# sczhou/CodeFormer

Measured on AMD Instinct MI355X. Metric: aligned 512x512 faces/sec (whole node) at w=0.5, higher is better.
Workload: dtype f32; 1 GPU; BASELINE config 2 (IEEE fp32 arithmetic): 16 faces/GPU, w=0.5, adain, seed-0 random-init weights; global_batch=16, parallelism=single GPU, precision=fp32

## Files before the change

### codeformer_amd/archs/codeformer_arch.py

```python
import gc
import os
import threading

import math
import numbers

import numpy as np
import torch
import torch.nn.functional as F
from torch import nn

from .. import ops
from ..ops import EPI_GELU, EPI_RESIDUAL, EPI_SFT, PRO_LEAKY
from ..utils.diagnostics import top2_gap
from ..utils.registry import ARCH_REGISTRY
from .hip_module import PACK_EPOCH, HipModule
from .vqgan_arch import ResBlock, VQAutoEncoder


_GRAPH_LOCK = threading.RLock()
_CAPTURE_STREAMS = {}


def _min_nan(a, b):
# ... 96 lines not shown
    normalized = (content_feat - content_mean.expand(size)) / content_std.expand(size)
    return normalized * style_std.expand(size) + style_mean.expand(size)


class TransformerSALayer(HipModule):

    def __init__(self, embed_dim, nhead=8, dim_mlp=2048, dropout=0.0, activation='gelu'):
        super().__init__()
        if activation != 'gelu':
            raise RuntimeError(f'activation should be gelu for the MI355X path, not {activation}.')
        self.self_attn = nn.MultiheadAttention(embed_dim, nhead, dropout=dropout)
        self.linear1 = nn.Linear(embed_dim, dim_mlp)
        self.dropout = nn.Dropout(dropout)
        self.linear2 = nn.Linear(dim_mlp, embed_dim)
        self.norm1 = nn.LayerNorm(embed_dim)
        self.norm2 = nn.LayerNorm(embed_dim)
        self.dropout1 = nn.Dropout(dropout)
        self.dropout2 = nn.Dropout(dropout)
        self.embed_dim, self.nhead = embed_dim, nhead

    def with_pos_embed(self, tensor, pos):
        return tensor if pos is None else tensor + pos

    def forward_tokens(self, X, pos, batch, code=0, code_ln=None):
        E, H = self.embed_dim, self.nhead
        sa = self.self_attn
        w, b = sa.in_proj_weight, sa.in_proj_bias
        code_ln = code if code_ln is None else code_ln
        c1 = ln_code(self, self.norm1, code_ln, pos)
        c2 = ln_code(self, self.norm2, code_ln)
        c_o = code or bounded_code(self, 'o', code_ln, self.norm1, w[2 * E:], b[2 * E:])
        c_d = code or bounded_code(self, 'd', code_ln, self.norm2, self.linear1.weight, self.linear1.bias)
        pw_o = self._pw_conv(sa.out_proj, bf16=c_o)
        if pos is not None:
            t2, t2p = ops.layernorm(X, self.norm1.weight, self.norm1.bias, self.norm1.eps, pos=pos)
        else:
            t2 = t2p = ops.layernorm(X, self.norm1.weight, self.norm1.bias, self.norm1.eps)
        if c1 == ops.GSPLIT and (2 * E) % 128 == 0:
            pw_qkv = self._packed(('qkv', c1), lambda: ops.pack_weight(w, b, bf16=c1), w, b)
            qkv = ops.linear(t2p, pw_qkv, x_alt=t2, alt_from=2 * E)
            q, k, v = qkv[:, :E], qkv[:, E:2 * E], qkv[:, 2 * E:]
        else:
            pw_qk = self._packed(('qk', c1), lambda: ops.pack_weight(w[:2 * E], b[:2 * E], bf16=c1), w, b)
            pw_v = self._packed(('v', c1), lambda: ops.pack_weight(w[2 * E:], b[2 * E:], bf16=c1), w, b)
            qk = ops.linear(t2p, pw_qk)
            v = ops.linear(t2, pw_v)
            q, k = qk[:, :E], qk[:, E:]
        hd = E // H
        a = ops.attention(q, k, v, batch, H, hd, float(hd) ** -0.5)
        X = ops.linear(a, pw_o, epilogue=EPI_RESIDUAL, res=X)
        t2 = ops.layernorm(X, self.norm2.weight, self.norm2.bias, self.norm2.eps)
        h = ops.linear(t2, self._pw_conv('linear1', bf16=c2), epilogue=EPI_GELU)
        return ops.linear(h, self._pw_conv('linear2', bf16=c_d), epilogue=EPI_RESIDUAL, res=X)

    def forward(self, tgt, tgt_mask=None, tgt_key_padding_mask=None, query_pos=None):
        if tgt.is_cuda:
            if tgt_mask is not None or tgt_key_padding_mask is not None:
                raise NotImplementedError('attention masks are not part of the CodeFormer inference path')
            with torch.no_grad():
                T, B, E = tgt.shape
                X = tgt.float().transpose(0, 1).contiguous().view(B * T, E)
# ... 82 lines not shown
@ARCH_REGISTRY.register()
class CodeFormer(VQAutoEncoder):

    def __init__(self, dim_embd=512, n_head=8, n_layers=9, codebook_size=1024, latent_size=256,
                 connect_list=['32', '64', '128', '256'], fix_modules=['quantize', 'generator'], vqgan_path=None):
        super().__init__(512, 64, [1, 2, 2, 4, 4, 8], 'nearest', 2, [16], codebook_size)
        if vqgan_path is not None:
            self.load_state_dict(torch.load(vqgan_path, map_location='cpu')['params_ema'])
        if fix_modules is not None:
            for name in fix_modules:
                for p in getattr(self, name).parameters():
                    p.requires_grad = False

        self.precision = os.environ.get('CODEFORMER_HIP_PRECISION', 'f16x2')
        self.bf16_storage = os.environ.get('CODEFORMER_HIP_BF16_STORAGE', '1') != '0'
        self.winograd_f43_encoder = os.environ.get('CODEFORMER_HIP_F43_ENCODER', '1') == '1'
        self.logit_guard = os.environ.get('CODEFORMER_HIP_LOGIT_GUARD', 'off')
        self.logit_guard_gap = float(os.environ.get('CODEFORMER_HIP_LOGIT_GUARD_GAP', '1.1e-4'))
        self.reset_guard_stats()
        self.encoder_precision = os.environ.get('CODEFORMER_HIP_ENCODER_PRECISION', 'auto')
        self.gemm_precision = os.environ.get('CODEFORMER_HIP_GEMM_PRECISION', 'auto')
        self.use_hip_graphs = {'0': False, '1': True}.get(os.environ.get('CODEFORMER_HIP_GRAPHS', 'auto'), 'auto')
        self.graph_max_batch = 4
        self._graphs = {}
        self.graph_captures = 0
        self.connect_list = connect_list
        self.n_layers = n_layers
        self.n_head = n_head
        self.dim_embd = dim_embd
        self.dim_mlp = dim_embd * 2
        self.latent_size = latent_size

        self.position_emb = nn.Parameter(torch.zeros(latent_size, self.dim_embd))
        self.feat_emb = nn.Linear(256, self.dim_embd)
        self.ft_layers = nn.Sequential(*[
            TransformerSALayer(embed_dim=dim_embd, nhead=n_head, dim_mlp=self.dim_mlp, dropout=0.0)
            for _ in range(self.n_layers)])
        self.idx_pred_layer = nn.Sequential(nn.LayerNorm(dim_embd), nn.Linear(dim_embd, codebook_size, bias=False))

        self.channels = {'16': 512, '32': 256, '64': 256, '128': 128, '256': 128, '512': 64}
        self.fuse_encoder_block = {'512': 2, '256': 5, '128': 8, '64': 11, '32': 14, '16': 18}
        self.fuse_generator_block = {'16': 6, '32': 9, '64': 12, '128': 15, '256': 18, '512': 21}
        self.fuse_convs_dict = nn.ModuleDict()
        for f_size in self.connect_list:
            ch = self.channels[f_size]
            self.fuse_convs_dict[f_size] = Fuse_sft_block(ch, ch)
# ... 4 lines not shown
        else:
            B, _, Himg, Wimg = x.shape
            if (Himg, Wimg) != (512, 512):
                raise ValueError(f'CodeFormer expects aligned 512x512 faces, got {Himg}x{Wimg}')
            x = x.float().contiguous()
        enc_feat = {}
        enc_taps = {self.fuse_encoder_block[f]: (lambda t: enc_feat.__setitem__(str(t.shape[2]), t))
                    for f in self.connect_list}
        if self.encoder_precision not in ('auto', 'fp32', 'f16x2'):
            raise ValueError(f"encoder_precision must be 'auto', 'fp32' or 'f16x2', got {self.encoder_precision!r}")
        enc_code = ops.SPLIT if self.encoder_precision == 'f16x2' or (self.encoder_precision == 'auto' and self.precision != 'fp32') else ops.WINOGRAD
        if self.winograd_f43_encoder if f43_encoder is None else f43_encoder:
            enc_code = {ops.SPLIT: ops.SPLIT_F43, ops.WINOGRAD: ops.WINOGRAD_F43K}[enc_code]
        lq = self.encoder.forward_nhwc(x, enc_taps, bf16=enc_code, img_u8=u8)
        T = lq.shape[1] * lq.shape[2]
        tokens = lq.view(B * T, lq.shape[3])

        if self.gemm_precision not in ('auto', 'fp32', 'f16x2'):
            raise ValueError(f"gemm_precision must be 'auto', 'fp32' or 'f16x2', got {self.gemm_precision!r}")
        gcode = ops.GSPLIT if self.gemm_precision == 'f16x2' else 0
        gcode_ln = ops.GSPLIT if (self.gemm_precision == 'f16x2' or (self.gemm_precision == 'auto' and self.precision != 'fp32' and self.encoder_precision != 'fp32')) else 0
        X = ops.linear(tokens, self._pw_conv('feat_emb', bf16=gcode))
        for layer in self.ft_layers:
            X = layer.forward_tokens(X, self.position_emb, B, code=gcode, code_ln=gcode_ln)
        ln, head = self.idx_pred_layer[0], self.idx_pred_layer[1]
        logits2d = ops.linear(ops.layernorm(X, ln.weight, ln.bias, ln.eps), self._pw_conv(head, bf16=ln_code(self, ln, gcode_ln)))
        res = {'logits': logits2d.view(B, T, -1), 'lq_feat': ops.to_nchw(lq), 'idx': None, 'quant': None, 'enc_feat': enc_feat}
        if guard:
            idx, _, self.last_min_gap = ops.argmax_rows_gap(logits2d, T)
            res['idx'] = idx.view(B, T)
        if code_only:
            return res

        if not guard:
            idx = ops.argmax_rows(logits2d)
            res['idx'] = idx.view(B, T)
        quant = ops.codebook_gather(idx, self.quantize.embedding.weight, B, T,
                                    lq=tokens.view(B, T, -1) if adain else None)
        res['quant'] = quant.view(B, lq.shape[1], lq.shape[2], -1)
        if self.precision not in ('fp32', 'f16x2', 'bf16', 'fp16'):
            raise ValueError(f"precision must be 'fp32', 'f16x2', 'bf16' or 'fp16', got {self.precision!r}")
        return res

    def _generate_hip(self, quant, enc_feat, w, u8=False, out_u8=None):
        B = quant.shape[0]
        bf16 = {'fp32': ops.WINOGRAD_F43K,'f16x2': ops.SPLIT_F43, 'bf16': 1, 'fp16': 2}[self.precision]
        gen_taps = None
# ... 76 lines not shown
            return self._generate_host(quant, enc_feat, w)
        if w.none_fused:
            return self._generate_host(quant, enc_feat, 0.0)
        wt = torch.tensor(w.host, dtype=torch.float32)
        if w.all_fused:
            return self._generate_host(quant, enc_feat, wt)
        rf, ru = w.rows_fused, w.rows_unfused
        of = self._generate_host(quant[rf], {f: t[rf] for f, t in enc_feat.items()}, wt[rf])
        ou = self._generate_host(quant[ru], None, 0.0)
        out = of.new_empty((quant.shape[0],) + tuple(of.shape[1:]))
        out[rf] = of
        out[ru] = ou
        return out

    def _forward_host(self, x, w, detach_16, code_only, adain):
        logits, lq_feat, quant, enc_feat = self._encode_host(x, detach_16, code_only, adain)
        if code_only:
            return logits, lq_feat
        return self._generate_rows_host(quant, enc_feat, w), logits, lq_feat

    def _forward_graphed(self, x, w, code_only, adain, guard=False, u8=False, out_u8=None):
        with _GRAPH_LOCK:
            per_face = isinstance(w, FaceWeights)
            key = (tuple(x.shape), ('per-face', w.fused) if per_face else float(w), bool(code_only), bool(adain), self.precision, bool(self.bf16_storage), self.encoder_precision, self.gemm_precision, bool(self.winograd_f43_encoder), str(x.device), ops.switches(), bool(guard), bool(u8))
            ent = self._graphs.get(key)
            sig = self._param_signature()
            if ent is None or ent['epoch'] != PACK_EPOCH[0] or ent['sig'] != sig:
                static_x = x.clone() if u8 else x.float().contiguous().clone()
                for _ in range(2):
                    self._forward_hip(static_x, w, code_only, adain, guard=guard, u8=u8)
                torch.cuda.synchronize(x.device)
                graph = torch.cuda.CUDAGraph()
                cap = _CAPTURE_STREAMS.get(str(x.device))
                if cap is None:
                    cap = _CAPTURE_STREAMS[str(x.device)] = torch.cuda.Stream(device=x.device)
                with torch.cuda.stream(cap):
                    ops._act_cells(x.device, 4 * max(int(x.shape[0]), 1))
                    ops._counters(x.device, 4096)
                    if self.precision == 'fp32':
                        ops._kpart_ws(x.device, max(int(x.shape[0]), 1) << 20)
                cap.synchronize()
                gc_on = gc.isenabled()
                gc.disable()
                try:
                    with torch.cuda.graph(graph, stream=cap):
                        outs = self._forward_hip(static_x, w, code_only, adain, guard=guard, u8=u8)
                finally:
# ... 240 lines not shown
```

### codeformer_amd/csrc/cf_conv_parts.h

```cpp
#pragma once
#include <type_traits>

#include "cf_common.h"

int cf_winograd_launch(const cf_conv_desc* d, hipStream_t stream, int* parts_query, const float* sft_w_img = nullptr);
bool cf_wsplit_covers(const cf_conv_desc* d);
int cf_wsplit_launch(const cf_conv_desc* d, hipStream_t stream, int* parts_query, const float* sft_w_img = nullptr);
int cf_wf43_launch(const cf_conv_desc* d, hipStream_t stream, int* parts_query, const float* sft_w_img = nullptr);
int cf_ksum_launch(const cf_conv_desc* d, hipStream_t stream, const float* sft_w_img);
bool cf_wf43_k32(int cout, int cin);
int cf_split_launch(const cf_conv_desc* d, hipStream_t stream, int* parts_query, const float* sft_w_img = nullptr);
int cf_gemm_split_launch(const cf_conv_desc* d, hipStream_t stream, int* parts_query);
int cf_gemm_f32_tile_try(const cf_conv_desc* d, hipStream_t stream);
int cf_gemm_split_geometry(const cf_conv_desc* d, int* tiles, long* bytes_per_part);
int cf_winograd_splitk_geometry(const cf_conv_desc* d, int* tiles, long* bytes_per_part);
int cf_split_splitk_geometry(const cf_conv_desc* d, int* tiles, long* bytes_per_part);

template <class A>
inline void cf_fill_conv_args(A& a, const cf_conv_desc* d, const float* sft_w_img = nullptr) {
  a.in0 = d->in0;
  a.in1 = d->in1;
  a.c0 = d->c0;
  a.c1 = d->c1;
  a.cin = d->c0 + d->c1;
  a.batch = d->batch;
  a.cout = d->cout;
  a.prologue = d->prologue;
  a.epilogue = d->epilogue;
  a.pro_scale = d->pro_scale;
  a.pro_shift = d->pro_shift;
  a.weight = d->weight;
  a.bias = d->bias;
  a.res = d->res;
  a.sft_scale = d->sft_scale;
  a.sft_w = d->sft_w;
  a.sft_w_img = sft_w_img;
// ... 156 lines not shown
```

### codeformer_amd/csrc/cf_gemm_split.hip

```cpp
#include <cstdlib>
#include <type_traits>

#include "cf_conv_parts.h"

namespace {

struct GsArgs {
  const float* a;
  const float* w;
  const float* bias;
  const float* res;
  float* out;
  int M, N, K;
  int epilogue;
  float acc_scale;
  float* ws;
  unsigned* counters;
  int nsplit;
  const float* a_alt;
  int n_alt;
};
__device__ __forceinline__ const float* gs_rows(const GsArgs& g, int n0) { return (g.a_alt && n0 >= g.n_alt) ? g.a_alt : g.a; }

__device__ __forceinline__ float gs_bias(const GsArgs& g, int n) { return g.bias ? g.bias[n] : 0.f; }
// ... 296 lines not shown
        for (int r = 0; r < 16; ++r) gs_part[(((c * MI + mi) * NI + ni) * 16 + r) * 64 + lane] = acc[mi][ni][r];
  }
  __syncthreads();
#pragma unroll
  for (int ni = 0; ni < NI; ++ni) {
    const int n = n0 + ni * 32 + l31;
    const float bias = gs_bias(g, n);
#pragma unroll
    for (int mi = 0; mi < MI; ++mi)
#pragma unroll
      for (int j = 0; j < 4; ++j) {
        const int r = wave + 4 * j;
        float tot = 0.f;
        for (int c = 0; c < V; ++c) tot += gs_part[(((c * MI + mi) * NI + ni) * 16 + r) * 64 + lane];
        const size_t o = (size_t)(m0 + mi * 32 + cf_acc_row(r, lane)) * g.N + n;
        float v = tot * g.acc_scale + bias;
        if (g.epilogue == CF_EPI_GELU) v = 0.5f * v * (1.0f + erff(v * 0.70710678118654752440f));
        if (g.epilogue == CF_EPI_RESIDUAL) v += g.res[o];
        g.out[o] = v;
      }
  }
}

__global__ __launch_bounds__(256) void gemm_f32_tile_kernel(const GsArgs g) {
  __shared__ __attribute__((aligned(16))) float As[2][2][128][16];
  const int tid = threadIdx.x, lane = tid & 63, wave = __builtin_amdgcn_readfirstlane(tid >> 6);
  const int wm = wave >> 1, wn = wave & 1;
  const int half = lane >> 5, l31 = lane & 31;
  const int ntn = g.N / 64;
  const int nt = blockIdx.x % ntn, mt = blockIdx.x / ntn;
  const int m0 = mt * 128, n0 = nt * 64 + wn * 32;
  const int nst = g.K >> 5;

  const float* const asrc = gs_rows(g, n0) + (size_t)(m0 + (tid >> 3)) * g.K + (tid & 7) * 4;
  f32x4 rg[4][4];
  auto load_stage = [&](int st, auto buf) __attribute__((always_inline)) {
    constexpr int BUF = decltype(buf)::value;
#pragma unroll
    for (int j = 0; j < 4; ++j) rg[BUF][j] = *reinterpret_cast<const f32x4*>(asrc + (size_t)(32 * j) * g.K + st * 32);
  };
  auto store_stage = [&](int lbuf, auto buf) __attribute__((always_inline)) {
    constexpr int BUF = decltype(buf)::value;
    const int q = tid & 7, ks = q >> 2, ch = q & 3;
#pragma unroll
    for (int j = 0; j < 4; ++j) {
      const int row = (tid >> 3) + 32 * j;
      *reinterpret_cast<f32x4*>(&As[lbuf][ks][row][(ch ^ ((row >> 2) & 3)) << 2]) = rg[BUF][j];
    }
  };
  const float* const wl = g.w + (size_t)(n0 + l31) * 16 + half * 4;
  const size_t kstride = (size_t)g.N * 16;
  f32x4 rb[4][2][2];
  auto load_B = [&](int st, auto buf) __attribute__((always_inline)) {
    constexpr int BUF = decltype(buf)::value;
#pragma unroll
    for (int s = 0; s < 2; ++s) {
      const float* p = wl + (size_t)(st * 2 + s) * kstride;
      rb[BUF][s][0] = *reinterpret_cast<const f32x4*>(p);
      rb[BUF][s][1] = *reinterpret_cast<const f32x4*>(p + 8);
    }
  };
  f32x16 acc[2], tot[2];
#pragma unroll
  for (int mi = 0; mi < 2; ++mi)
#pragma unroll
    for (int r = 0; r < 16; ++r) acc[mi][r] = tot[mi][r] = 0.f;
  auto compute = [&](int lbuf, auto buf) __attribute__((always_inline)) {
    constexpr int BUF = decltype(buf)::value;
#pragma unroll
    for (int s = 0; s < 2; ++s) {
      f32x4 a0[2], a1[2];
#pragma unroll
      for (int mi = 0; mi < 2; ++mi) {
        const int row = wm * 64 + mi * 32 + l31;
        const int swz = (row >> 2) & 3;
        a0[mi] = *reinterpret_cast<const f32x4*>(&As[lbuf][s][row][(half ^ swz) << 2]);
        a1[mi] = *reinterpret_cast<const f32x4*>(&As[lbuf][s][row][((2 + half) ^ swz) << 2]);
      }
#pragma unroll
      for (int j = 0; j < 4; ++j)
#pragma unroll
        for (int mi = 0; mi < 2; ++mi) acc[mi] = __builtin_amdgcn_mfma_f32_32x32x2f32(a0[mi][j], rb[BUF][s][0][j], acc[mi], 0, 0, 0);
#pragma unroll
      for (int j = 0; j < 4; ++j)
#pragma unroll
        for (int mi = 0; mi < 2; ++mi) acc[mi] = __builtin_amdgcn_mfma_f32_32x32x2f32(a1[mi][j], rb[BUF][s][1][j], acc[mi], 0, 0, 0);
    }
  };
  using R0 = std::integral_constant<int, 0>;
  using R1 = std::integral_constant<int, 1>;
  using R2 = std::integral_constant<int, 2>;
  using R3 = std::integral_constant<int, 3>;
  auto stage = [&](int st, auto cur, auto nxt, auto far, auto do_load, auto do_store) __attribute__((always_inline)) {
    if constexpr (decltype(do_load)::value) {
      load_stage(st + 3, far);
      load_B(st + 3, far);
    }
    __builtin_amdgcn_sched_barrier(0);
    compute(st & 1, cur);
    if ((st & 3) == 3) {
#pragma unroll
      for (int mi = 0; mi < 2; ++mi) {
        tot[mi] += acc[mi];
#pragma unroll
        for (int r = 0; r < 16; ++r) acc[mi][r] = 0.f;
      }
    }
    if constexpr (decltype(do_store)::value) store_stage((st + 1) & 1, nxt);
    __syncthreads();
  };
  constexpr std::true_type Y{};
  constexpr std::false_type NO{};
  load_stage(0, R0{});
  load_B(0, R0{});
  load_stage(1, R1{});
  load_B(1, R1{});
  load_stage(2, R2{});
  load_B(2, R2{});
  store_stage(0, R0{});
  __syncthreads();
  int st = 0;
  for (; st + 4 < nst; st += 4) {
    stage(st, R0{}, R1{}, R3{}, Y, Y);
    stage(st + 1, R1{}, R2{}, R0{}, Y, Y);
    stage(st + 2, R2{}, R3{}, R1{}, Y, Y);
    stage(st + 3, R3{}, R0{}, R2{}, Y, Y);
  }
  stage(st, R0{}, R1{}, R3{}, Y, Y);
  stage(st + 1, R1{}, R2{}, R0{}, NO, Y);
  stage(st + 2, R2{}, R3{}, R1{}, NO, Y);
  stage(st + 3, R3{}, R0{}, R2{}, NO, NO);

  const int n = n0 + l31;
  const float bias = gs_bias(g, n);
#pragma unroll
  for (int mi = 0; mi < 2; ++mi)
#pragma unroll
    for (int r = 0; r < 16; ++r) gs_finish<false>(g, tot[mi][r], m0 + wm * 64 + mi * 32 + cf_acc_row(r, lane), n, bias);
}

bool gs_plain_token_gemm(const cf_conv_desc* d) {
  return d->stride == 1 && !d->in_nchw && !d->out_nchw && d->c1 == 0 && d->prologue == CF_PRO_NONE && !d->stats_out &&
         (d->ld_in0 == 0 || d->ld_in0 == d->c0) && (d->ld_out == 0 || d->ld_out == d->cout);
}
bool gs_epi_known(const cf_conv_desc* d) { return d->epilogue == CF_EPI_NONE || d->epilogue == CF_EPI_GELU || d->epilogue == CF_EPI_RESIDUAL; }

GsArgs gs_args(const cf_conv_desc* d, long m, int nsplit, float* ws, unsigned* counters, const float* a_alt) {
  GsArgs g;
  g.a = d->in0;
  g.w = d->weight;
  g.bias = d->bias;
  g.res = d->res;
  g.out = d->out;
  g.M = (int)m;
  g.N = d->cout;
  g.K = d->c0;
  g.epilogue = d->epilogue;
  g.acc_scale = d->acc_scale;
  g.ws = ws;
  g.counters = counters;
  g.nsplit = nsplit;
// ... 38 lines not shown
    CF_LDS_ATTR((gemm_split_chunk_kernel<1, 1>), GS_CHUNK_MAXV * 4096);
    hipLaunchKernelGGL((gemm_split_chunk_kernel<1, 1>), dim3((unsigned)((g.M / 32) * (g.N / 32))), dim3(256), (size_t)V * 4096, stream, g);
    CF_CHECK_LAUNCH("cf_conv2d(1x1, f16x2, in-workgroup split)");
    return CF_OK;
  }
  const int nsplit = d->split_k >= 1 ? d->split_k : 1;
  CF_REQUIRE(V % nsplit == 0, "cf_conv2d(1x1, f16x2): split_k %d must divide K/128 = %d", nsplit, V);
  CF_REQUIRE(nsplit == 1 || (d->workspace && d->counters), "cf_conv2d(1x1, f16x2): split_k > 1 needs workspace and counters");
  if (parts_query) {
    *parts_query = 0;
    return CF_OK;
  }
  const GsArgs g = gs_args(d, m, nsplit, d->workspace, d->counters, d->in0_alt);
  if (nsplit == 1 && g.M % 128 == 0 && g.K % 64 == 0) {
    hipLaunchKernelGGL(gemm_split_tile_kernel<1>, dim3((unsigned)((g.M / 128) * (g.N / 64))), dim3(256), 0, stream, g);
    CF_CHECK_LAUNCH("cf_conv2d(1x1, f16x2, token tiles)");
    return CF_OK;
  }
  hipLaunchKernelGGL(gemm_split_kernel, dim3((unsigned)(tiles * nsplit)), dim3(256), 0, stream, g);
  CF_CHECK_LAUNCH("cf_conv2d(1x1, f16x2)");
  return CF_OK;
}

int cf_gemm_f32_tile_try(const cf_conv_desc* d, hipStream_t stream) {
  const long m = (long)d->batch * d->hout * d->wout;
  const int k = d->c0;
  if (d->taps != 1 || d->bf16_mfma != CF_OPERAND_F32 || d->split_k != 1 || !gs_plain_token_gemm(d) || !gs_epi_known(d) || d->stats_cpg ||
      m % 128 || k % 128 || d->cout % 64 || d->cout_pad != d->cout || d->pad_mode != CF_PAD_ZERO)
    return 1;
  if (k == 512 && d->cout == 512) return 1;
  const GsArgs g = gs_args(d, m, 1, nullptr, nullptr, nullptr);
  hipLaunchKernelGGL(gemm_f32_tile_kernel, dim3((unsigned)((g.M / 128) * (g.N / 64))), dim3(256), 0, stream, g);
  CF_CHECK_LAUNCH("cf_conv2d(1x1, fp32 token tiles)");
  return CF_OK;
}
```

### codeformer_amd/csrc/cf_igemm.hip

```cpp
#include <string.h>
#include <type_traits>

#include "cf_conv_parts.h"

namespace {

struct ConvArgs {
  const float* in0;
  const float* in1;
  int c0, c1, cin, nchunks;
  int batch, hin, win, hout, wout;
  int cout, cout_pad;
  int upsample, out_nchw, prologue, epilogue;
  const float* pro_scale;
  const float* pro_shift;
  const float* weight;
  const float* bias;
  const float* res;
  const float* sft_scale;
  const float* sft_w_img;
  float* out;
  double* stats_out;
  int stats_cpg, nparts;
  int tiles_x, tiles_per_img, ntn;
// ... 1117 lines not shown
  CF_REQUIRE(d->pad_lo == 0 || d->stride == 2, "cf_conv2d: pad_lo applies to stride 2");
  const bool ext = !d->winograd && d->bf16_mfma != CF_OPERAND_F16X2 && (ld0 != d->c0 || ld1 != d->c1 || ldo != d->cout || d->epilogue >= CF_EPI_LEAKY ||
                   ((d->pad_mode != CF_PAD_ZERO || d->pad_lo) && !(d->out_nchw && d->cout <= 4)) ||
                   (d->bf16_mfma == CF_OPERAND_F16 && d->cout_pad % 64 != 0) ||
                   (d->taps == 9 && d->stride == 1 && !d->in_nchw && !few_cout && (d->hout % 16 != 0 || d->wout % 16 != 0)) ||
                   (d->upsample && d->bf16_mfma == CF_OPERAND_F32 && d->cout_pad % 128 == 0 && (d->hin % 8 != 0 || d->win % 16 != 0)));
  if (ext) {
    CF_REQUIRE(d->taps == 9 && (d->stride == 1 || (d->bf16_mfma == CF_OPERAND_F32 && d->cout_pad % 128 == 0)) && !d->in_nchw &&
                   !d->out_nchw && d->bf16_mfma != CF_OPERAND_BF16 && !d->stats_out &&
                   !(pq && d->stats_cpg) && d->cout % 4 == 0 && d->epilogue != CF_EPI_SFT && d->epilogue != CF_EPI_GELU,
               "cf_conv2d: strided slices / leaky|axpy epilogues / off-grid sizes (%dx%d) need a 3x3 stride-1 fp32 / f16-operand NHWC conv with "
               "cout %% 4 == 0, no statistics, epilogue in {none, residual, leaky, axpy, axpy2, prelu, res_prelu}", d->hout, d->wout);
    CF_REQUIRE(ld0 % 4 == 0 && ld1 % 4 == 0 && ldo % 4 == 0, "cf_conv2d: channel strides must be multiples of 4 floats");
    CF_REQUIRE(d->epilogue < CF_EPI_PRELU || (d->bf16_mfma == CF_OPERAND_F32 && !d->upsample),
               "cf_conv2d: the PReLU epilogues are built for plain 3x3 convs with fp32 operands (operand %d, upsample %d)", d->bf16_mfma, d->upsample);
  } else {
    CF_REQUIRE(!few_cout || ld0 == d->c0, "cf_conv2d: the NCHW <=4-channel output conv reads a dense input");
    CF_REQUIRE(d->epilogue < CF_EPI_PRELU, "cf_conv2d: the PReLU epilogues belong to the general fp32 / f16-operand 3x3 instantiations (winograd %d, operand %d)",
               d->winograd, d->bf16_mfma);
  }
  CF_REQUIRE(!(d->out_nchw && (d->taps != 9 || d->epilogue != CF_EPI_NONE)), "cf_conv2d: out_nchw needs 3x3, no epilogue");
  CF_REQUIRE(d->cout_pad >= d->cout && d->cout_pad % 32 == 0, "cf_conv2d: cout_pad %d invalid for cout %d", d->cout_pad,
             d->cout);
  CF_REQUIRE(!d->in0_alt || (d->taps == 1 && d->bf16_mfma == CF_OPERAND_F16X2 && (long)d->hout * d->wout <= CF_TOKEN_IMAGE_MAX && !d->io_bf16),
             "cf_conv2d: in0_alt (a second token matrix for the columns >= alt_cout0) belongs to the split-half token GEMM");
  if (d->io_bf16) {
    const bool dense = ld0 == d->c0 && ld1 == d->c1 && ldo == d->cout && d->pad_mode == CF_PAD_ZERO && !d->in_nchw && d->stride == 1 && d->split_k < 1;
    const bool wino_bf16 = d->winograd == 1 && d->bf16_mfma == CF_OPERAND_BF16;
    const bool direct_bf16 = !d->winograd && d->bf16_mfma == CF_OPERAND_BF16 && d->taps == 9 && !d->out_nchw &&
                             (d->upsample ? (d->cout_pad % 128 == 0 && (long)d->hout * d->wout > 1024) : d->cout_pad == 64);
    const bool conv1 = !d->winograd && d->bf16_mfma == CF_OPERAND_F32 && d->taps == 1 && (d->cout_pad % 128 == 0 || d->cout_pad == 64) &&
                       (long)d->hout * d->wout > 1024;
    const bool conv1s = !d->winograd && d->bf16_mfma == CF_OPERAND_F16X2 && d->taps == 1 && (long)d->hout * d->wout > CF_TOKEN_IMAGE_MAX;
    const bool head = few_cout && d->bf16_mfma == CF_OPERAND_F32 && !d->winograd && d->cout == 3;
    CF_REQUIRE(d->io_bf16 == 1 && dense && !ext && (head || d->cout % 4 == 0) && (wino_bf16 || direct_bf16 || conv1 || conv1s || head),
               "cf_conv2d: io_bf16 (bf16 tensors) is built for dense stride-1 launches of the bf16 mode: winograd + CF_OPERAND_BF16, direct CF_OPERAND_BF16 3x3 "
               "(cout_pad 64) / folded upsample (cout_pad %% 128 == 0), fp32 1x1 on images of more than 1024 pixels, the 3-channel NCHW head "
               "(taps %d operand %d winograd %d cout_pad %d upsample %d)", d->taps, d->bf16_mfma, d->winograd, d->cout_pad, d->upsample);
    CF_REQUIRE(d->epilogue == CF_EPI_NONE || d->epilogue == CF_EPI_RESIDUAL || d->epilogue == CF_EPI_SFT, "cf_conv2d: io_bf16 epilogues are none / residual / SFT");
  }
  if (d->act_scale) {
    CF_REQUIRE(d->prologue == CF_PRO_NONE || d->prologue == CF_PRO_LEAKY,
               "cf_conv2d: act_scale is for un-normalised inputs (prologue none / leaky), got prologue %d", d->prologue);
    const bool conv1x1_split = d->taps == 1 && d->bf16_mfma == CF_OPERAND_F16X2 && (long)d->hout * d->wout > CF_TOKEN_IMAGE_MAX;
    CF_REQUIRE((d->taps == 9 && (d->bf16_mfma == CF_OPERAND_F32 || d->winograd || d->bf16_mfma == CF_OPERAND_F16X2)) || conv1x1_split,
               "cf_conv2d: act_scale is applied by the Winograd / split-half convolution kernels only (operand %d, winograd %d, taps %d)",
               d->bf16_mfma, d->winograd, d->taps);
  }
// ... 240 lines not shown
```

### codeformer_amd/ops.py

```python
import ctypes
import math
import os
import weakref

import torch

from . import lib as L
from .lib import (EPI_AXPY, EPI_AXPY2, EPI_GELU, EPI_LEAKY, EPI_NONE, EPI_PRELU, EPI_RES_PRELU, EPI_RESIDUAL, EPI_SFT, PRO_AFFINE, PRO_AFFINE_SWISH,
                  PAD_EDGE, PAD_REFLECT, PAD_ZERO, PRO_LEAKY, PRO_NONE)

GN_GROUPS = 32
GN_EPS = 1e-6

PROFILE = None


def _f32(t):
    if t.dtype != torch.float32:
        raise TypeError(f'expected float32, got {t.dtype}')
    return t


def _act_dtype(t, what='activation'):
    if t.dtype not in (torch.float32, torch.bfloat16):
# ... 441 lines not shown


def splitk_for(pw, ho, wo, cin, batch=1):
    if (pw.bf16 and not pw.wino and pw.taps != 1) or ho * wo > 1024 or cin % 128:
        return 0
    if pw.wino == 2:
        return 0
    if pw.wino:
        if ho % 8 or wo % 16 or ho * wo > 256:
            return 0
        tiles = batch * (ho // 8) * (wo // 16) * (pw.cout_pad // 64)
    elif pw.taps == 1 and (ho * wo) % 64 == 0 and pw.cout_pad % 64 == 0:
        if int(pw.bf16) == OPERAND_F16X2 and not pw.conv1 and batch * ho * wo * pw.cout_pad <= GEMM_IN_WG_MAX_OUTPUTS and cin <= 1024:
            return SPLITK_IN_WORKGROUP
        tiles = batch * (ho * wo // 64) * (pw.cout_pad // 64)
    else:
        return 0
    cap = 256 if pw.wino else 128
    v = cin // 128
    for ns in (8, 4, 2):
        if ns <= SPLITK_MAX and v % ns == 0 and tiles * ns <= cap:
            return ns
    return 1


def _counters(device, n):
    return _scratch(_COUNTERS, device, n, 4096)


_KPART_WS = {}


def _kpart_ws(device, n):
    return _scratch(_KPART_WS, device, n, 1 << 22)


def _roofline_kind(pw, io, stride, upsample, c0, in_nchw, out_nchw, out_pixels, split_k):
    kind = ('conv3x3_s2' if stride == 2 else ('conv_up2x' if upsample else ('conv3x3_wino' if pw.wino else 'conv3x3'))) if pw.taps == 9 else 'gemm1x1'
    if pw.taps == 9 and stride == 1 and ((in_nchw and c0 <= 4) or (out_nchw and pw.cout <= 4)):
        kind = 'conv3x3_io'
    if pw.bf16:
        kind += ('', '_bf16', '_f16', '_f16x2')[int(pw.bf16)]
    if io == torch.bfloat16 and not pw.bf16:
        kind += '_bf16io'
    if pw.conv1:
        kind = 'conv1x1_stream_f16x2'
# ... 80 lines not shown
        if t is not None and _nhwc_ld(t, 'epilogue operand') != (ldo or pw.cout):
            raise ValueError('epilogue operands must have the channel stride of the output')
    for t in (scale, shift):
        if t is not None and tuple(t.shape) != (B, c0 + c1):
            raise ValueError(f'prologue table shape {tuple(t.shape)} != {(B, c0 + c1)}')
    w_img = None
    if torch.is_tensor(sft_w):
        if epilogue != EPI_SFT or u8_in is not None or u8_out is not None:
            raise ValueError('sft_w: a tensor (one weight per image) belongs to epilogue=EPI_SFT; the other epilogues take a float')
        if sft_w.dtype != torch.float32:
            raise TypeError(f'sft_w: expected a float32 tensor of {B} values, got {sft_w.dtype}')
        if sft_w.dim() != 1 or sft_w.shape[0] != B or sft_w.device != dev:
            raise ValueError(f'sft_w: expected {B} values (one per image) on {dev}, got shape {tuple(sft_w.shape)} on {sft_w.device}')
        w_img, sft_w = L.ptr(sft_w), 0.0
    d = L.ConvDesc(
        in0=None if img_in is not None else L.ptr(x, not in_nchw, dtype=io), in1=L.ptr(x2, True, dtype=io), c0=c0, c1=c1, batch=B, hin=H, win=W, hout=Ho, wout=Wo, cout=pw.cout,
        cout_pad=pw.cout_pad, taps=pw.taps, stride=stride, upsample=2 if f42_up else int(bool(upsample)), in_nchw=int(bool(in_nchw)),
        out_nchw=int(bool(out_nchw)), prologue=prologue, epilogue=epilogue, pro_scale=L.ptr(scale),
        pro_shift=L.ptr(shift), weight=L.ptr(pw.w, dtype=None), bias=L.ptr(pw.bias), res=L.ptr(res, True, dtype=io),
        sft_scale=L.ptr(sft_scale, True, dtype=io), sft_w=float(sft_w), out=None if img_out is not None else L.ptr(out, not out_nchw, dtype=odt), bf16_mfma=int(pw.bf16),
        ld_in0=ld0, ld_in1=ld1, ld_out=ldo, pad_mode=int(pad_mode), pad_lo=int(pad_lo), winograd=int(pw.wino),
        acc_scale=1.0 / pw.scale, io_bf16=int(io == torch.bfloat16))
    if x_alt is not None:
        if tuple(x_alt.shape) != tuple(x.shape) or x_alt.dtype != torch.float32 or int(pw.bf16) != OPERAND_F16X2 or pw.taps != 1 or pw.conv1 or x2 is not None:
            raise ValueError('x_alt: a second float32 token matrix of the same shape, for a split-half token GEMM (bf16=GSPLIT weight)')
        d.in0_alt, d.alt_cout0 = L.ptr(x_alt), int(alt_from)
    if act is not None and needs_act_scale(pw):
        if tuple(act.shape) != (B, 2) or prologue not in (PRO_NONE, PRO_LEAKY):
            raise ValueError('act: expected a (B, 2) table and a none / leaky prologue')
        d.act_scale = L.ptr(act)
    if pw.kparts:
        dense = not in_nchw and not out_nchw and ld0 == c0 and (c1 == 0 or ld1 == c1) and ldo in (0, pw.cout)
        if split_k or upsample or stride != 1 or not dense or io != torch.float32 or not f43k_covers(c0 + c1, pw.cout, Ho, Wo, c0 if c1 else None):
            raise ValueError('a weight packed with bf16=WF43K serves dense fp32 3x3 stride-1 launches of the shapes f43k_covers names (conv_code decides: pack with its answer)')
        d.split_k = pw.kparts
        d.workspace = L.ptr(_kpart_ws(dev, pw.kparts * B * Ho * Wo * pw.cout), dtype=torch.int32)
        split_k = 0
    elif split_k is None:
        dense = not in_nchw and not out_nchw and ld0 == c0 and (c1 == 0 or ld1 == c1) and ldo in (0, pw.cout)
        split_k = splitk_for(pw, Ho, Wo, c0 + c1, B) if (stride == 1 and dense) else 0
    if split_k:
        d.split_k = int(split_k)
        if split_k > 1:
            nbytes, tiles = lib.cf_conv2d_workspace_bytes(ctypes.byref(d)), lib.cf_conv2d_tiles(ctypes.byref(d))
            if nbytes < 0 or tiles <= 0:
                raise RuntimeError(f'cf_conv2d_workspace_bytes failed: {L.last_error()}')
            ws = torch.empty(nbytes // 4, dtype=torch.float32, device=dev)
            d.workspace, d.counters = L.ptr(ws), L.ptr(_counters(dev, tiles), dtype=torch.int32)
# ... 22 lines not shown
    if PROFILE is None:
        launch()
        return out
    e0, e1 = torch.cuda.Event(enable_timing=True), torch.cuda.Event(enable_timing=True)
    e0.record()
    launch()
    e1.record()
    x = img_in if img_in is not None else x
    cin = c0 + c1
    flops = 2.0 * B * Ho * Wo * pw.cout * cin * (4 if (upsample and not pw.wino) else pw.taps)
    esz = x.element_size()
    nbytes = float(esz * (x.numel() + (0 if x2 is None else x2.numel()) + (0 if res is None else res.numel()) + (0 if sft_scale is None else sft_scale.numel()))
                   + 4 * pw.cout * cin * pw.taps + out.element_size() * out.numel())
    kind = _roofline_kind(pw, io, stride, upsample, c0, in_nchw, out_nchw, Ho * Wo, split_k)
    PROFILE.append((kind, flops, nbytes, e0, e1, (B, H, W, cin, pw.cout)))
    return out


def linear(x, pw, *, epilogue=EPI_NONE, res=None, x_alt=None, alt_from=0):
    M, K = x.shape
    if M % 256:
        raise ValueError(f'linear: rows {M} must be a multiple of 256')
    r4 = None if res is None else res.view(M // 256, 16, 16, pw.cout)
    y = conv2d(x.view(M // 256, 16, 16, K), pw, epilogue=epilogue, res=r4, x_alt=None if x_alt is None else x_alt.view(M // 256, 16, 16, K), alt_from=alt_from)
    return y.view(M, pw.cout)


FINALIZE_FUSED = os.environ.get('CODEFORMER_HIP_FINALIZE_FUSED', '1') != '0'


def groupnorm_tables(xs, gamma, beta, eps=GN_EPS, groups=GN_GROUPS, act_growth=None):
    lib = L.load()
    B, H, W, _ = xs[0].shape
    ctot = sum(t.shape[3] for t in xs)
    if ctot % groups:
        raise ValueError(f'{ctot} channels not divisible by {groups} groups')
    cpg = ctot // groups
    hw = H * W
    dev = xs[0].device
    scale = torch.empty(B, ctot, dtype=torch.float32, device=dev)
    shift = torch.empty_like(scale)
    g_ptr, b_ptr, sc_ptr, sh_ptr = L.ptr(gamma), L.ptr(beta), L.ptr(scale), L.ptr(shift)
    stats = []
    for t in xs:
        _act_dtype(t)
        c = t.shape[3]
        if c % cpg:
# ... 937 lines not shown
```

Measured before the change: 360.0 faces/s.

## Fuse fp32 QKV projection into one launch with 64-row token-tile GEMM kernel

In the fp32 GEMM path, the transformer's Q/K and V projections now run as one fused QKV GEMM. It reads the pos-added LayerNorm output for the Q/K columns and the plain one for the V columns, where before this took two launches. The fp32 token-tile kernel is rewritten from 128x64 tiles to 64x64 tiles. It uses a single accumulator per wave, a shallower prefetch pipeline, launch_bounds occupancy 4, and support for the alternate input matrix. The old 512x512 exclusion is also dropped, so more GEMMs use this kernel. The aim is fewer launches and better occupancy and grid fill on small token GEMMs, at the cost of less register-level reuse per tile.

```diff
diff --git a/codeformer_amd/archs/codeformer_arch.py b/codeformer_amd/archs/codeformer_arch.py
--- a/codeformer_amd/archs/codeformer_arch.py
+++ b/codeformer_amd/archs/codeformer_arch.py
@@ -142,7 +142,7 @@
     def with_pos_embed(self, tensor, pos):
         return tensor if pos is None else tensor + pos
 
-    def forward_tokens(self, X, pos, batch, code=0, code_ln=None):
+    def forward_tokens(self, X, pos, batch, code=0, code_ln=None, qkv_one_launch=True):
         E, H = self.embed_dim, self.nhead
         sa = self.self_attn
         w, b = sa.in_proj_weight, sa.in_proj_bias
@@ -156,7 +156,11 @@
             t2, t2p = ops.layernorm(X, self.norm1.weight, self.norm1.bias, self.norm1.eps, pos=pos)
         else:
             t2 = t2p = ops.layernorm(X, self.norm1.weight, self.norm1.bias, self.norm1.eps)
-        if c1 == ops.GSPLIT and (2 * E) % 128 == 0:
+        if c1 == 0 and qkv_one_launch and (2 * E) % 128 == 0 and all(ops.f32_tile_takes(n, E, batch) for n in (3 * E, 2 * E, E)):
+            pw_qkv = self._packed(('qkv', 0), lambda: ops.pack_weight(w, b), w, b)
+            qkv = ops.linear(t2p, pw_qkv, x_alt=t2, alt_from=2 * E)
+            q, k, v = qkv[:, :E], qkv[:, E:2 * E], qkv[:, 2 * E:]
+        elif c1 == ops.GSPLIT and (2 * E) % 128 == 0:
             pw_qkv = self._packed(('qkv', c1), lambda: ops.pack_weight(w, b, bf16=c1), w, b)
             qkv = ops.linear(t2p, pw_qkv, x_alt=t2, alt_from=2 * E)
             q, k, v = qkv[:, :E], qkv[:, E:2 * E], qkv[:, 2 * E:]
@@ -285,6 +289,7 @@
         self.gemm_precision = os.environ.get('CODEFORMER_HIP_GEMM_PRECISION', 'auto')
         self.use_hip_graphs = {'0': False, '1': True}.get(os.environ.get('CODEFORMER_HIP_GRAPHS', 'auto'), 'auto')
         self.graph_max_batch = 4
+        self.qkv_one_launch = True
         self._graphs = {}
         self.graph_captures = 0
         self.connect_list = connect_list
@@ -335,7 +340,7 @@
         gcode_ln = ops.GSPLIT if (self.gemm_precision == 'f16x2' or (self.gemm_precision == 'auto' and self.precision != 'fp32' and self.encoder_precision != 'fp32')) else 0
         X = ops.linear(tokens, self._pw_conv('feat_emb', bf16=gcode))
         for layer in self.ft_layers:
-            X = layer.forward_tokens(X, self.position_emb, B, code=gcode, code_ln=gcode_ln)
+            X = layer.forward_tokens(X, self.position_emb, B, code=gcode, code_ln=gcode_ln, qkv_one_launch=self.qkv_one_launch)
         ln, head = self.idx_pred_layer[0], self.idx_pred_layer[1]
         logits2d = ops.linear(ops.layernorm(X, ln.weight, ln.bias, ln.eps), self._pw_conv(head, bf16=ln_code(self, ln, gcode_ln)))
         res = {'logits': logits2d.view(B, T, -1), 'lq_feat': ops.to_nchw(lq), 'idx': None, 'quant': None, 'enc_feat': enc_feat}
@@ -458,7 +463,7 @@
     def _forward_graphed(self, x, w, code_only, adain, guard=False, u8=False, out_u8=None):
         with _GRAPH_LOCK:
             per_face = isinstance(w, FaceWeights)
-            key = (tuple(x.shape), ('per-face', w.fused) if per_face else float(w), bool(code_only), bool(adain), self.precision, bool(self.bf16_storage), self.encoder_precision, self.gemm_precision, bool(self.winograd_f43_encoder), str(x.device), ops.switches(), bool(guard), bool(u8))
+            key = (tuple(x.shape), ('per-face', w.fused) if per_face else float(w), bool(code_only), bool(adain), self.precision, bool(self.bf16_storage), self.encoder_precision, self.gemm_precision, bool(self.winograd_f43_encoder), str(x.device), ops.switches(), bool(guard), bool(u8), bool(self.qkv_one_launch))
             ent = self._graphs.get(key)
             sig = self._param_signature()
             if ent is None or ent['epoch'] != PACK_EPOCH[0] or ent['sig'] != sig:
diff --git a/codeformer_amd/csrc/cf_conv_parts.h b/codeformer_amd/csrc/cf_conv_parts.h
--- a/codeformer_amd/csrc/cf_conv_parts.h
+++ b/codeformer_amd/csrc/cf_conv_parts.h
@@ -12,6 +12,7 @@
 int cf_split_launch(const cf_conv_desc* d, hipStream_t stream, int* parts_query, const float* sft_w_img = nullptr);
 int cf_gemm_split_launch(const cf_conv_desc* d, hipStream_t stream, int* parts_query);
 int cf_gemm_f32_tile_try(const cf_conv_desc* d, hipStream_t stream);
+bool cf_gemm_f32_tile_takes(const cf_conv_desc* d);
 int cf_gemm_split_geometry(const cf_conv_desc* d, int* tiles, long* bytes_per_part);
 int cf_winograd_splitk_geometry(const cf_conv_desc* d, int* tiles, long* bytes_per_part);
 int cf_split_splitk_geometry(const cf_conv_desc* d, int* tiles, long* bytes_per_part);
diff --git a/codeformer_amd/csrc/cf_gemm_split.hip b/codeformer_amd/csrc/cf_gemm_split.hip
--- a/codeformer_amd/csrc/cf_gemm_split.hip
+++ b/codeformer_amd/csrc/cf_gemm_split.hip
@@ -342,69 +342,60 @@
   }
 }
 
-__global__ __launch_bounds__(256) void gemm_f32_tile_kernel(const GsArgs g) {
-  __shared__ __attribute__((aligned(16))) float As[2][2][128][16];
+__global__ __launch_bounds__(256, 4) void gemm_f32_tile64_kernel(const GsArgs g) {
+  __shared__ __attribute__((aligned(16))) float As[2][2][64][16];
   const int tid = threadIdx.x, lane = tid & 63, wave = __builtin_amdgcn_readfirstlane(tid >> 6);
   const int wm = wave >> 1, wn = wave & 1;
   const int half = lane >> 5, l31 = lane & 31;
   const int ntn = g.N / 64;
   const int nt = blockIdx.x % ntn, mt = blockIdx.x / ntn;
-  const int m0 = mt * 128, n0 = nt * 64 + wn * 32;
+  const int m0 = mt * 64, n0 = nt * 64 + wn * 32;
   const int nst = g.K >> 5;
 
-  const float* const asrc = gs_rows(g, n0) + (size_t)(m0 + (tid >> 3)) * g.K + (tid & 7) * 4;
-  f32x4 rg[4][4];
+  const float* const abase = gs_rows(g, nt * 64) + (size_t)m0 * g.K;
+  const unsigned aoff = (unsigned)((tid >> 3) * g.K + (tid & 7) * 4) * 4u;
+  f32x4 rg[4][2];
   auto load_stage = [&](int st, auto buf) __attribute__((always_inline)) {
     constexpr int BUF = decltype(buf)::value;
 #pragma unroll
-    for (int j = 0; j < 4; ++j) rg[BUF][j] = *reinterpret_cast<const f32x4*>(asrc + (size_t)(32 * j) * g.K + st * 32);
+    for (int j = 0; j < 2; ++j) rg[BUF][j] = *reinterpret_cast<const f32x4*>(reinterpret_cast<const char*>(abase + (size_t)(32 * j) * g.K + st * 32) + aoff);
   };
   auto store_stage = [&](int lbuf, auto buf) __attribute__((always_inline)) {
     constexpr int BUF = decltype(buf)::value;
     const int q = tid & 7, ks = q >> 2, ch = q & 3;
 #pragma unroll
-    for (int j = 0; j < 4; ++j) {
+    for (int j = 0; j < 2; ++j) {
       const int row = (tid >> 3) + 32 * j;
       *reinterpret_cast<f32x4*>(&As[lbuf][ks][row][(ch ^ ((row >> 2) & 3)) << 2]) = rg[BUF][j];
     }
   };
-  const float* const wl = g.w + (size_t)(n0 + l31) * 16 + half * 4;
+  const float* const wbase = g.w + (size_t)(nt * 64) * 16;
+  const unsigned woff = (unsigned)((wn * 32 + l31) * 16 + half * 4) * 4u;
   const size_t kstride = (size_t)g.N * 16;
   f32x4 rb[4][2][2];
   auto load_B = [&](int st, auto buf) __attribute__((always_inline)) {
     constexpr int BUF = decltype(buf)::value;
 #pragma unroll
     for (int s = 0; s < 2; ++s) {
-      const float* p = wl + (size_t)(st * 2 + s) * kstride;
+      const float* p = reinterpret_cast<const float*>(reinterpret_cast<const char*>(wbase + (size_t)(st * 2 + s) * kstride) + woff);
       rb[BUF][s][0] = *reinterpret_cast<const f32x4*>(p);
       rb[BUF][s][1] = *reinterpret_cast<const f32x4*>(p + 8);
     }
   };
-  f32x16 acc[2], tot[2];
-#pragma unroll
-  for (int mi = 0; mi < 2; ++mi)
-#pragma unroll
-    for (int r = 0; r < 16; ++r) acc[mi][r] = tot[mi][r] = 0.f;
+  f32x16 acc, tot;
+#pragma unroll
+  for (int r = 0; r < 16; ++r) acc[r] = tot[r] = 0.f;
+  const int arow = wm * 32 + l31, aswz = (arow >> 2) & 3;
   auto compute = [&](int lbuf, auto buf) __attribute__((always_inline)) {
     constexpr int BUF = decltype(buf)::value;
 #pragma unroll
     for (int s = 0; s < 2; ++s) {
-      f32x4 a0[2], a1[2];
-#pragma unroll
-      for (int mi = 0; mi < 2; ++mi) {
-        const int row = wm * 64 + mi * 32 + l31;
-        const int swz = (row >> 2) & 3;
-        a0[mi] = *reinterpret_cast<const f32x4*>(&As[lbuf][s][row][(half ^ swz) << 2]);
-        a1[mi] = *reinterpret_cast<const f32x4*>(&As[lbuf][s][row][((2 + half) ^ swz) << 2]);
-      }
-#pragma unroll
-      for (int j = 0; j < 4; ++j)
-#pragma unroll
-        for (int mi = 0; mi < 2; ++mi) acc[mi] = __builtin_amdgcn_mfma_f32_32x32x2f32(a0[mi][j], rb[BUF][s][0][j], acc[mi], 0, 0, 0);
-#pragma unroll
-      for (int j = 0; j < 4; ++j)
-#pragma unroll
-        for (int mi = 0; mi < 2; ++mi) acc[mi] = __builtin_amdgcn_mfma_f32_32x32x2f32(a1[mi][j], rb[BUF][s][1][j], acc[mi], 0, 0, 0);
+      const f32x4 a0 = *reinterpret_cast<const f32x4*>(&As[lbuf][s][arow][(half ^ aswz) << 2]);
+      const f32x4 a1 = *reinterpret_cast<const f32x4*>(&As[lbuf][s][arow][((2 + half) ^ aswz) << 2]);
+#pragma unroll
+      for (int j = 0; j < 4; ++j) acc = __builtin_amdgcn_mfma_f32_32x32x2f32(a0[j], rb[BUF][s][0][j], acc, 0, 0, 0);
+#pragma unroll
+      for (int j = 0; j < 4; ++j) acc = __builtin_amdgcn_mfma_f32_32x32x2f32(a1[j], rb[BUF][s][1][j], acc, 0, 0, 0);
     }
   };
   using R0 = std::integral_constant<int, 0>;
@@ -412,19 +403,14 @@
   using R2 = std::integral_constant<int, 2>;
   using R3 = std::integral_constant<int, 3>;
   auto stage = [&](int st, auto cur, auto nxt, auto far, auto do_load, auto do_store) __attribute__((always_inline)) {
-    if constexpr (decltype(do_load)::value) {
-      load_stage(st + 3, far);
-      load_B(st + 3, far);
-    }
+    if constexpr (decltype(do_load)::value) load_B(st + 2, far);
+    if constexpr (decltype(do_store)::value) load_stage(st + 1, nxt);
     __builtin_amdgcn_sched_barrier(0);
     compute(st & 1, cur);
     if ((st & 3) == 3) {
-#pragma unroll
-      for (int mi = 0; mi < 2; ++mi) {
-        tot[mi] += acc[mi];
-#pragma unroll
-        for (int r = 0; r < 16; ++r) acc[mi][r] = 0.f;
-      }
+      tot += acc;
+#pragma unroll
+      for (int r = 0; r < 16; ++r) acc[r] = 0.f;
     }
     if constexpr (decltype(do_store)::value) store_stage((st + 1) & 1, nxt);
     __syncthreads();
@@ -433,30 +419,28 @@
   constexpr std::false_type NO{};
   load_stage(0, R0{});
   load_B(0, R0{});
-  load_stage(1, R1{});
   load_B(1, R1{});
-  load_stage(2, R2{});
-  load_B(2, R2{});
   store_stage(0, R0{});
   __syncthreads();
   int st = 0;
   for (; st + 4 < nst; st += 4) {
-    stage(st, R0{}, R1{}, R3{}, Y, Y);
-    stage(st + 1, R1{}, R2{}, R0{}, Y, Y);
-    stage(st + 2, R2{}, R3{}, R1{}, Y, Y);
-    stage(st + 3, R3{}, R0{}, R2{}, Y, Y);
-  }
-  stage(st, R0{}, R1{}, R3{}, Y, Y);
-  stage(st + 1, R1{}, R2{}, R0{}, NO, Y);
-  stage(st + 2, R2{}, R3{}, R1{}, NO, Y);
-  stage(st + 3, R3{}, R0{}, R2{}, NO, NO);
-
-  const int n = n0 + l31;
+    stage(st, R0{}, R1{}, R2{}, Y, Y);
+    stage(st + 1, R1{}, R2{}, R3{}, Y, Y);
+    stage(st + 2, R2{}, R3{}, R0{}, Y, Y);
+    stage(st + 3, R3{}, R0{}, R1{}, Y, Y);
+  }
+  stage(st, R0{}, R1{}, R2{}, Y, Y);
+  stage(st + 1, R1{}, R2{}, R3{}, Y, Y);
+  stage(st + 2, R2{}, R3{}, R0{}, NO, Y);
+  stage(st + 3, R3{}, R0{}, R1{}, NO, NO);
+
+  int t2 = tid;
+  asm volatile("" : "+v"(t2));
+  const int lane2 = t2 & 63, wave2 = __builtin_amdgcn_readfirstlane(t2 >> 6);
+  const int n = nt * 64 + (wave2 & 1) * 32 + (lane2 & 31);
   const float bias = gs_bias(g, n);
 #pragma unroll
-  for (int mi = 0; mi < 2; ++mi)
-#pragma unroll
-    for (int r = 0; r < 16; ++r) gs_finish<false>(g, tot[mi][r], m0 + wm * 64 + mi * 32 + cf_acc_row(r, lane), n, bias);
+  for (int r = 0; r < 16; ++r) gs_finish<false>(g, tot[r], m0 + (wave2 >> 1) * 32 + cf_acc_row(r, lane2), n, bias);
 }
 
 bool gs_plain_token_gemm(const cf_conv_desc* d) {
@@ -541,15 +525,19 @@
   return CF_OK;
 }
 
+bool cf_gemm_f32_tile_takes(const cf_conv_desc* d) {
+  const long m = (long)d->batch * d->hout * d->wout;
+  if (d->taps != 1 || d->bf16_mfma != CF_OPERAND_F32 || d->split_k != 1 || !gs_plain_token_gemm(d) || !gs_epi_known(d) || d->stats_cpg ||
+      m % 128 || d->c0 % 128 || d->cout % 64 || d->cout_pad != d->cout || d->pad_mode != CF_PAD_ZERO)
+    return false;
+  return !d->in0_alt || (d->alt_cout0 > 0 && d->alt_cout0 < d->cout && d->alt_cout0 % 128 == 0);
+}
+
 int cf_gemm_f32_tile_try(const cf_conv_desc* d, hipStream_t stream) {
+  if (!cf_gemm_f32_tile_takes(d)) return 1;
   const long m = (long)d->batch * d->hout * d->wout;
-  const int k = d->c0;
-  if (d->taps != 1 || d->bf16_mfma != CF_OPERAND_F32 || d->split_k != 1 || !gs_plain_token_gemm(d) || !gs_epi_known(d) || d->stats_cpg ||
-      m % 128 || k % 128 || d->cout % 64 || d->cout_pad != d->cout || d->pad_mode != CF_PAD_ZERO)
-    return 1;
-  if (k == 512 && d->cout == 512) return 1;
-  const GsArgs g = gs_args(d, m, 1, nullptr, nullptr, nullptr);
-  hipLaunchKernelGGL(gemm_f32_tile_kernel, dim3((unsigned)((g.M / 128) * (g.N / 64))), dim3(256), 0, stream, g);
+  const GsArgs g = gs_args(d, m, 1, nullptr, nullptr, d->in0_alt);
+  hipLaunchKernelGGL(gemm_f32_tile64_kernel, dim3((unsigned)((g.M / 64) * (g.N / 64))), dim3(256), 0, stream, g);
   CF_CHECK_LAUNCH("cf_conv2d(1x1, fp32 token tiles)");
   return CF_OK;
 }
diff --git a/codeformer_amd/csrc/cf_igemm.hip b/codeformer_amd/csrc/cf_igemm.hip
--- a/codeformer_amd/csrc/cf_igemm.hip
+++ b/codeformer_amd/csrc/cf_igemm.hip
@@ -1163,8 +1163,10 @@
   CF_REQUIRE(!(d->out_nchw && (d->taps != 9 || d->epilogue != CF_EPI_NONE)), "cf_conv2d: out_nchw needs 3x3, no epilogue");
   CF_REQUIRE(d->cout_pad >= d->cout && d->cout_pad % 32 == 0, "cf_conv2d: cout_pad %d invalid for cout %d", d->cout_pad,
              d->cout);
-  CF_REQUIRE(!d->in0_alt || (d->taps == 1 && d->bf16_mfma == CF_OPERAND_F16X2 && (long)d->hout * d->wout <= CF_TOKEN_IMAGE_MAX && !d->io_bf16),
-             "cf_conv2d: in0_alt (a second token matrix for the columns >= alt_cout0) belongs to the split-half token GEMM");
+  CF_REQUIRE(!d->in0_alt || (d->taps == 1 && (long)d->hout * d->wout <= CF_TOKEN_IMAGE_MAX && !d->io_bf16 &&
+                             (d->bf16_mfma == CF_OPERAND_F16X2 || (!pq && !d->winograd && cf_gemm_f32_tile_takes(d)))),
+             "cf_conv2d: in0_alt (a second token matrix for the columns >= alt_cout0) belongs to the split-half token GEMM and, with fp32 operands, to "
+             "the token-tile GEMM (split_k 1, M %% 128 == 0, K %% 128 == 0, cout %% 64 == 0 == cout_pad - cout, 0 < alt_cout0 < cout a multiple of 128)");
   if (d->io_bf16) {
     const bool dense = ld0 == d->c0 && ld1 == d->c1 && ldo == d->cout && d->pad_mode == CF_PAD_ZERO && !d->in_nchw && d->stride == 1 && d->split_k < 1;
     const bool wino_bf16 = d->winograd == 1 && d->bf16_mfma == CF_OPERAND_BF16;
diff --git a/codeformer_amd/ops.py b/codeformer_amd/ops.py
--- a/codeformer_amd/ops.py
+++ b/codeformer_amd/ops.py
@@ -487,6 +487,11 @@
         if ns <= SPLITK_MAX and v % ns == 0 and tiles * ns <= cap:
             return ns
     return 1
+
+
+def f32_tile_takes(cout, cin, batch, ho=16, wo=16):
+    pw = PackedWeight(None, None, cout, cin, 1, _cout_pad(cout), cin)
+    return pw.cout_pad == cout and cout % 64 == 0 and cin % 128 == 0 and (batch * ho * wo) % 128 == 0 and splitk_for(pw, ho, wo, cin, batch) == 1
 
 
 def _counters(device, n):
@@ -613,8 +618,10 @@
         ld_in0=ld0, ld_in1=ld1, ld_out=ldo, pad_mode=int(pad_mode), pad_lo=int(pad_lo), winograd=int(pw.wino),
         acc_scale=1.0 / pw.scale, io_bf16=int(io == torch.bfloat16))
     if x_alt is not None:
-        if tuple(x_alt.shape) != tuple(x.shape) or x_alt.dtype != torch.float32 or int(pw.bf16) != OPERAND_F16X2 or pw.taps != 1 or pw.conv1 or x2 is not None:
-            raise ValueError('x_alt: a second float32 token matrix of the same shape, for a split-half token GEMM (bf16=GSPLIT weight)')
+        if tuple(x_alt.shape) != tuple(x.shape) or x_alt.dtype != torch.float32 or int(pw.bf16) not in (OPERAND_F16X2, 0) or pw.wino or pw.taps != 1 or pw.conv1 or x2 is not None:
+            raise ValueError('x_alt: a second float32 token matrix of the same shape, for a token GEMM (a bf16=GSPLIT weight, or an fp32 one on a launch f32_tile_takes)')
+        if not pw.bf16 and split_k != 1:
+            raise ValueError('x_alt with an fp32 weight: pass split_k=1 (the token-tile launch, where f32_tile_takes; no other fp32 kernel reads x_alt)')
         d.in0_alt, d.alt_cout0 = L.ptr(x_alt), int(alt_from)
     if act is not None and needs_act_scale(pw):
         if tuple(act.shape) != (B, 2) or prologue not in (PRO_NONE, PRO_LEAKY):
@@ -683,7 +690,8 @@
     if M % 256:
         raise ValueError(f'linear: rows {M} must be a multiple of 256')
     r4 = None if res is None else res.view(M // 256, 16, 16, pw.cout)
-    y = conv2d(x.view(M // 256, 16, 16, K), pw, epilogue=epilogue, res=r4, x_alt=None if x_alt is None else x_alt.view(M // 256, 16, 16, K), alt_from=alt_from)
+    sk = 1 if (x_alt is not None and not pw.bf16) else None
+    y = conv2d(x.view(M // 256, 16, 16, K), pw, epilogue=epilogue, res=r4, x_alt=None if x_alt is None else x_alt.view(M // 256, 16, 16, K), alt_from=alt_from, split_k=sk)
     return y.view(M, pw.cout)
 
 
```

After: 360.8 faces/s, median of 6. No clear change (+0.2%).
